# shepherdvovkes/sparse-matrix-multiplication-benchmark

Hardware: AMD Instinct MI355X
Metric: TCSC SpMM: effective G-add-ops/s + achieved HBM GB/s vs roofline, 1/2/4/8 GPU (higher is better)
Workload: dtype f32; 1 GPU; cfg4: M=4096 K=16384 N=16384, 98% ternary sparsity, fp32, tcsc_gemm_prelu; M=4096, K=16384, N=16384, variant=prelu_basic, columns_per_gpu=16384, nnz_per_gpu=5369271, parallelism=column-shard x1 (strong), no collective, rows_per_gpu=4096

## Files before the change

### include/tcsc_gpu.h

```cpp
#ifndef TCSC_AMD_TCSC_GPU_H
#define TCSC_AMD_TCSC_GPU_H

#include <stddef.h>
#include "sparse/tcsc.h"

#ifdef __cplusplus
extern "C" {
#endif

enum tcsc_variant {
    TCSC_VARIANT_BASIC = 0,
    TCSC_VARIANT_OPTIMIZED = 1,
    TCSC_VARIANT_PRELU_BASIC = 2,
    TCSC_VARIANT_PRELU_SEPARATE = 3,
    TCSC_VARIANT_PRELU_ONTHEGO = 4,
    TCSC_VARIANT_SPARSE_GEMM = 5
};

enum tcsc_status {
    TCSC_OK = 0,
    TCSC_E_ARG = 1,
    TCSC_E_HIP = 2,
    TCSC_E_NOMEM = 3,
    TCSC_E_NODEV = 4
// ... 39 lines not shown
int tcsc_gpu_plan_get_info(const tcsc_gpu_plan *plan, tcsc_gpu_plan_info *info);

enum tcsc_path {
    TCSC_PATH_GATHER = 0,
    TCSC_PATH_FUSED = 1,
    TCSC_PATH_MFMA = 2,
    TCSC_PATH_SMALL = 3,
    TCSC_PATH_DECODE = 4
};
int tcsc_gpu_launch_info(const tcsc_gpu_plan *plan, int M, int *path, int *slices);

int tcsc_gpu_launch_combine(const tcsc_gpu_plan *plan, int M, int *in_launch);

int tcsc_gpu_launch_geometry(const tcsc_gpu_plan *plan, int M, int *cols_per_wave);
int tcsc_gpu_wide_pays(int M, int ncols, int num_cus);

int tcsc_gpu_plan_reserve(tcsc_gpu_plan *plan, int max_M);
void tcsc_gpu_plan_destroy(tcsc_gpu_plan *plan);

#define TCSC_PATH_AUTO (-1)
int tcsc_gpu_plan_workspace(const tcsc_gpu_plan *plan, int M, int path, size_t *need, size_t *reserved);

int tcsc_gpu_sgemm(const tcsc_gpu_plan *plan, const float *dX, const float *dB,
                   float *dY, int M, int ldy, int variant, float a,
                   void *stream);

int tcsc_gpu_prepare_x(const tcsc_gpu_plan *plan, const float *dX, int M, void *stream);
int tcsc_gpu_sgemm_prepared(const tcsc_gpu_plan *plan, const float *dB, float *dY, int M, int ldy,
                            int variant, float a, void *stream);

// ... 98 lines not shown
```

### sparse-matrix-multiplication-benchmark_amd/csrc/tcsc_api.cpp

```cpp
#include <hip/hip_runtime.h>
#include <rocblas/rocblas.h>

#include <algorithm>
#include <cstdarg>
#include <cstdint>
#include <cstdio>
#include <cstdlib>
#include <cstring>
#include <memory>
#include <mutex>
#include <string>
#include <unordered_map>
#include <vector>

#include "../../include/sparse/tcsc.h"
#include "../../include/tcsc_gpu.h"
#include "tcsc_plan.h"

struct tcsc_gpu_plan {
    int device = 0;
    int rows = 0, cols = 0, col_begin = 0;
    long long n_pos = 0, n_neg = 0;
    int n_chunks = 0, n_groups = 0;
    long long n_entries = 0;
// ... 10 lines not shown
    size_t mfma_bytes = 0;
    int8_t* w8 = nullptr;
    size_t i8_bytes = 0;
    uint32_t* w2 = nullptr;
    size_t w2_bytes = 0;
    int *ccq = nullptr, *crq = nullptr;
    size_t csc_bytes = 0;
    int mfma_min_M = 0;
    unsigned* csync = nullptr;
    mutable bool csync_dirty = false;
    int num_cus = 0;
    int2* ent_w = nullptr;
    int* sptr_w = nullptr;
    long long n_entries_w = 0;
    int n_groups_w = 0;
    size_t wide_bytes = 0;
    float* tbias = nullptr;
    size_t tbias_bytes = 0;
    bool packed = false;
};

namespace {
thread_local std::string g_last_error;
}

namespace tcsc {

void set_error(const char* fmt, ...) {
    char buf[512];
    va_list ap;
// ... 560 lines not shown
    if (f == tcsc::kWideCW) return true;
    if (f == tcsc::kCW) return false;
    const int top = std::min(max_M, kMaxLaunchRows);
    for (long long M = tcsc::kTM; M < top + tcsc::kTM; M += tcsc::kTM)
        if (wide_pays((int)std::min<long long>(M, top), p->cols, p->num_cus)) return true;
    return false;
}

int build_wide(tcsc_gpu_plan* p) {
    if (p->ent_w) return TCSC_OK;
    DeviceGuard dg(p->device);
    hipStream_t st = nullptr;
    const int nch = p->n_chunks, G = p->n_groups, ncols = p->cols, Gw = tcsc::wide_groups_for(ncols);
    const long long nc = (long long)nch * ncols, ng = (long long)nch * Gw;
    if (nch <= 0 || ng + 1 > 0x7fffffffLL) return TCSC_OK;
    DevBuf cnt, cptr, gcnt, tmp;
    size_t tb1 = 0, tb2 = 0;
    HIP_TRY(tcsc::plan_scan_tmp_bytes(nc + 1, &tb1));
    HIP_TRY(tcsc::plan_scan_tmp_bytes(ng + 1, &tb2));
    const size_t tb = std::max(tb1, tb2);
    int* sptr_w = nullptr;
    if (cnt.alloc((size_t)(nc + 1) * sizeof(int)) != hipSuccess || cptr.alloc((size_t)(nc + 1) * sizeof(int)) != hipSuccess ||
        gcnt.alloc((size_t)(ng + 1) * sizeof(int)) != hipSuccess || tmp.alloc(tb) != hipSuccess ||
        hipMalloc(&sptr_w, (size_t)(ng + 1) * sizeof(int)) != hipSuccess) {
        (void)hipGetLastError();
        return TCSC_OK;
    }
    std::unique_ptr<int, void (*)(int*)> sptr_guard(sptr_w, [](int* q) { (void)hipFree(q); });
    HIP_TRY(hipDeviceSynchronize());
    HIP_TRY(tcsc::wide_counts(p->ent, p->sptr, G, nch, ncols, Gw, cnt.as<int>(), cptr.as<int>(), gcnt.as<int>(), sptr_w,
                              tmp.p, tb, st));
    int total = 0;
    HIP_TRY(hipMemcpyAsync(&total, sptr_w + ng, sizeof(int), hipMemcpyDeviceToHost, st));
    HIP_TRY(hipStreamSynchronize(st));
    int2* ent_w = nullptr;
    if (hipMalloc(&ent_w, (size_t)(total + tcsc::kEntGuard) * sizeof(int2)) != hipSuccess) {
        (void)hipGetLastError();
        return TCSC_OK;
    }
    hipError_t e = tcsc::wide_fill(p->ent, p->sptr, G, nch, ncols, Gw, cptr.as<int>(), sptr_w, ent_w, total, st);
    if (e == hipSuccess) e = hipStreamSynchronize(st);
    if (e != hipSuccess) {
        (void)hipFree(ent_w);
        return hip_fail(e, "build_wide");
    }
    p->ent_w = ent_w;
    p->sptr_w = sptr_guard.release();
    p->n_entries_w = total;
    p->n_groups_w = Gw;
    p->wide_bytes = (size_t)(ng + 1) * sizeof(int) + (size_t)(total + tcsc::kEntGuard) * sizeof(int2);
    return TCSC_OK;
}

int launch_geo(const tcsc_gpu_plan* p, int M, int slices, int forced_slices, const char* who) {
    const int f = geo_override();
    if (f == tcsc::kWideCW) {
        if (p->order != TCSC_ORDER_FAST || forced_slices > 1) {
            if (who)
                set_error("%s: TCSC_GEO=22 needs the fast order and an unsplit K (order %s, %d slices forced)", who,
                          p->order == TCSC_ORDER_FAST ? "fast" : "reference", forced_slices);
            return -1;
        }
        if (p->rows <= 0) return tcsc::kCW;
        if (!p->ent_w) {
            if (who)
// ... 214 lines not shown
        g.ent2 = p->chain_neg->ent;
        g.sptr2 = p->chain_neg->sptr;
        g.n_entries2 = p->chain_neg->n_entries;
    }
    g.n_groups = p->n_groups;
    g.a = a;
    g.slices = r.slices;
    g.combine = r.combine;
    g.stage = stage;
    if (stage != 1) {
        if (r.geo < 0) return TCSC_E_ARG;
        if (r.geo == tcsc::kWideCW) {
            g.geo = r.geo;
            g.ent = p->ent_w;
            g.sptr = p->sptr_w;
            g.n_entries = p->n_entries_w;
            g.n_groups = p->n_groups_w;
            g.slices = 1;
            g.combine = 0;
        }
    }
    if (pins.plan_ws && p->csync) {
        if (p->csync_dirty) {
            HIP_TRY(hipMemsetAsync(p->csync, 0, tcsc::kCombineBytes, static_cast<hipStream_t>(stream)));
            p->csync_dirty = false;
        }
        g.ccnt = p->csync;
        g.combine_giveup = combine_giveup_knob();
    }
    g.bias_first = (g.order == 1 && variant == TCSC_VARIANT_BASIC);
// ... 459 lines not shown
    g_order = order == TCSC_ORDER_REFERENCE ? TCSC_ORDER_REFERENCE : TCSC_ORDER_FAST;
}

int tcsc_gpu_get_order(void) { return current_order(); }

void tcsc_gpu_plan_destroy(tcsc_gpu_plan* p) {
    if (!p) return;
    DeviceGuard dg(p->device);
    if (p->ent) (void)hipFree(p->ent);
    if (p->sptr) (void)hipFree(p->sptr);
    if (p->ws) (void)hipFree(p->ws);
    if (p->csync) (void)hipFree(p->csync);
    if (p->tbias) (void)hipFree(p->tbias);
    if (p->ent_w) (void)hipFree(p->ent_w);
    if (p->sptr_w) (void)hipFree(p->sptr_w);
    free_mfma(p);
    free_csc(p);
    tcsc_gpu_plan_destroy(p->chain_pos);
    tcsc_gpu_plan_destroy(p->chain_neg);
    delete p;
}

int tcsc_gpu_plan_reserve(tcsc_gpu_plan* p, int max_M) {
    if (!p || max_M < 0) {
        set_error("tcsc_gpu_plan_reserve: bad arguments");
        return TCSC_E_ARG;
    }
    const size_t want = reserve_bytes(p, max_M);
    if (!p->csync && p->rows > 0 && p->order == TCSC_ORDER_FAST && !p->packed) {
        DeviceGuard dg(p->device);
// ... 48 lines not shown
}

int tcsc_gpu_launch_info(const tcsc_gpu_plan* p, int M, int* path, int* slices) {
    return launch_info_impl("tcsc_gpu_launch_info", p, M, path, slices, kF32);
}

int tcsc_gpu_launch_info_bf16(const tcsc_gpu_plan* p, int M, int* path, int* slices) {
    return launch_info_impl("tcsc_gpu_launch_info_bf16", p, M, path, slices, kBf16);
}

int tcsc_gpu_launch_info_i8(const tcsc_gpu_plan* p, int M, int* path, int* slices) {
    return launch_info_impl("tcsc_gpu_launch_info_i8", p, M, path, slices, kI8);
}

int tcsc_gpu_wide_pays(int M, int ncols, int num_cus) { return wide_pays(M, ncols, num_cus) ? 1 : 0; }

int tcsc_gpu_launch_geometry(const tcsc_gpu_plan* p, int M, int* cols_per_wave) {
    if (!p || M < 0 || !cols_per_wave) {
        set_error("tcsc_gpu_launch_geometry: bad arguments");
        return TCSC_E_ARG;
    }
    if (refuse_packed(p, "tcsc_gpu_launch_geometry")) return TCSC_E_ARG;
    *cols_per_wave = 0;
    const Route r = plan_route(p, M, kF32, "tcsc_gpu_launch_geometry");
    if (r.path != TCSC_PATH_GATHER) return TCSC_OK;
    if (r.geo < 0) return TCSC_E_ARG;
    *cols_per_wave = r.geo;
    return TCSC_OK;
}

// ... 601 lines not shown
```

### sparse-matrix-multiplication-benchmark_amd/csrc/tcsc_internal.h

```cpp
#pragma once
#include <hip/hip_runtime.h>
#include <stddef.h>
#include <stdint.h>

namespace tcsc {

constexpr int kTM = 256;
#ifndef TCSC_TK
#define TCSC_TK 48
#endif
#ifndef TCSC_NBUF
#define TCSC_NBUF 3
#endif
constexpr int kTK = TCSC_TK;
constexpr int kNBuf = TCSC_NBUF;
constexpr int kRowBytes = kTM * 4;
constexpr int kBufRows = kTK + 1;
#ifndef TCSC_WAVES
#define TCSC_WAVES 16
#endif
#ifndef TCSC_CW
#define TCSC_CW 16
#endif
#ifndef TCSC_BATCH
// ... 60 lines not shown
constexpr int kDmaPerWave = kTK / kDmaWaves;
static_assert(kDmaWaves <= kWaves && kTK % kDmaWaves == 0, "each DMA wave moves the same number of rows");
static_assert(kLdsBytes <= 160 * 1024, "LDS");
static_assert(kNBuf >= 2 && kNBuf <= 5, "ring of 2 (DMA(c+1) before gather(c)) or n >= 3 (DMA(c+n-1) after it)");

static_assert(4 * kCW <= 255, "slot index must fit the 8-bit gpr_idx field");
static_assert(64 * 16 <= 1024, "lane byte offset (16*lane) must fit the 10 low address bits");

constexpr int kWideCW = 22;
constexpr int kWideBatch = 3;
constexpr int kWideWgCols = kWaves * kWideCW;
__host__ __device__ constexpr int wide_group_col0(int g) { return (g / kWaves) * kWideWgCols + (g % kWaves) * kWideCW; }
__host__ __device__ constexpr int wide_groups_for(int ncols) {
    return (ncols / kWideWgCols) * kWaves + (ncols % kWideWgCols + kWideCW - 1) / kWideCW;
}

struct PlanDev {
    int rows = 0;
    int ncols = 0;
    int col_begin = 0;
    long long n_pos = 0, n_neg = 0;
    const int* csp = nullptr;
    const int* csn = nullptr;
    const int* rip = nullptr;
    const int* rin = nullptr;
};

struct PlanOut {
    int n_chunks = 0;
    int n_groups = 0;
// ... 18 lines not shown
struct GemmArgs {
    const void* X = nullptr;
    int xtype = kF32;
    const float* Xscale = nullptr;
    float* XT = nullptr;
    int M = 0, K = 0;
    const int2* ent = nullptr;
    const int* sptr = nullptr;
    long long n_entries = 0;
    int order = 0;
    const int2* ent2 = nullptr;
    const int* sptr2 = nullptr;
    long long n_entries2 = 0;
    int n_groups = 0;
    int geo = kCW;
    int ncols = 0;
    const float* B = nullptr;
    float* Y = nullptr;
    int ldy = 0;
    float a = 0.f;
    bool bias_first = false;
    bool prelu = false;
    float* ws = nullptr;
    size_t ws_bytes = 0;
    int slices = 1;
    int combine = 0;
    int stage = 0;
    unsigned* ccnt = nullptr;
    int combine_giveup = 0;
};
// ... 2 lines not shown
           ((reinterpret_cast<uintptr_t>(g.Y) | reinterpret_cast<uintptr_t>(g.ws) | reinterpret_cast<uintptr_t>(g.B)) & 15) == 0;
}
constexpr int kMaxLaunchRows = 1 << 22;

hipError_t plan_scan_tmp_bytes(long long n, size_t* bytes);
hipError_t plan_counts(const PlanDev& in, PlanOut& out, hipStream_t st);
hipError_t plan_fill(const PlanDev& in, PlanOut& out, hipStream_t st);
int choose_slices(int M, int ncols, int K, long long nnz, int n_groups, size_t ws_bytes, int force);
int combine_mode(int slices, long long wgs, long long tiles, long long slab_floats, int num_cus, bool have_words,
                 bool vec);
int normalized_slices(int K, int slices);
void pf_stream_params(long long n_entries, int n_groups, int n_chunks, int* dist, int* lines);
size_t workspace_bytes(int M, int ncols, int slices);
size_t xt_bytes(int M, int K);
hipError_t launch_gemm(const GemmArgs& g, hipStream_t st);
hipError_t wide_counts(const int2* ent, const int* sptr, int G, int nch, int ncols, int Gw, int* cnt, int* cptr,
                       int* gcnt, int* sptr_w, void* tmp, size_t tmp_bytes, hipStream_t st);
hipError_t wide_fill(const int2* ent, const int* sptr, int G, int nch, int ncols, int Gw, const int* cptr,
                     const int* sptr_w, int2* ent_w, long long n_entries, hipStream_t st);
hipError_t launch_stream_wide(const GemmArgs& g, hipStream_t st);
int dense_tile_rows(int rows);
hipError_t dense_to_tcsc_counts(const float* D, int rows, int cols, int* cp, int* cn, int* totp, int* totn,
                                hipStream_t st);
hipError_t dense_to_tcsc_fill(const float* D, int rows, int cols, const int* csp, const int* csn, const int* op,
                              const int* on, int* rip, int* rin, hipStream_t st);
hipError_t launch_bias_act(float* Y, int M, int N, int ldy, const float* B, bool prelu, float a, hipStream_t st);
hipError_t exclusive_scan_i32(const int* in, int* out, int n, void* tmp, size_t tmp_bytes, hipStream_t st);
hipError_t check_index_device(const int* cs, const int* ri, int col_begin, int ncols, int rows, int n_total,
                              int* d_flag, hipStream_t st);
hipError_t rebase_offsets(const int* cs, int col_begin, int ncols, int* out, hipStream_t st);
hipError_t sort_columns_tmp_bytes(int n, int ncols, size_t* bytes);
hipError_t sort_columns(const int* in, int* out, int n, int ncols, const int* off, void* tmp, size_t tmp_bytes,
                        hipStream_t st);
int ldxt_for(int M);
// ... 125 lines not shown
```

### sparse-matrix-multiplication-benchmark_amd/csrc/tcsc_wide.hip

```cpp
#include <hip/hip_runtime.h>
#include <hipcub/hipcub.hpp>
#include <stdint.h>

#include "tcsc_internal.h"

namespace tcsc {

#include "gather_asm_w22.inc"

static_assert(TCSCW_GEN_CW == kWideCW && TCSCW_GEN_BATCH == kWideBatch, "generated loop geometry");
static_assert(TCSCW_GEN_CAP + kHdr <= kEntGuard, "stream prefetch stays inside the entry guard");
static_assert(TCSCW_GEN_HDR == 2 * kHdr, "generated loop and plan agree on the chunk header");
static_assert(TCSCW_GEN_BUDGET == (512 / kWavesPerSimd) / 8 * 8, "generated loop VGPR budget");
static_assert(TCSCW_GEN_TAIL == 1, "the wide streams are unpadded");
static_assert(TCSCW_GEN_TOUCH == 0 && TCSCW_GEN_PF == 0, "no scalar-cache touches in the wide loop");
static_assert(4 * kWideCW <= 255, "slot index must fit the 8-bit gpr_idx field");
static_assert(kWaves == 16 && kTK % 16 == 0 && kNBuf >= 3, "the wide kernel's DMA split and ring");

namespace {

typedef float f32x32_t __attribute__((ext_vector_type(32)));
typedef float f32x16_t __attribute__((ext_vector_type(16)));
typedef float f32x8_t __attribute__((ext_vector_type(8)));
constexpr int kAccWidths[] = {TCSCW_ACC_WIDTHS};
// ... 81 lines not shown

__device__ __forceinline__ void xcd_tile_w(int bx, int by, int ncb, int nrt, int& cb, int& rt) {
    const int T = ncb * nrt;
    const int L = bx + ncb * by;
    const int q = T >> 3, r = T & 7, x = L & 7;
    const int Lg = (x < r ? x * (q + 1) : r * (q + 1) + (x - r) * q) + (L >> 3);
    cb = Lg % ncb;
    rt = Lg / ncb;
}

constexpr int kEpiRowsW = 64;
constexpr int kStrideW = kWideWgCols * 4 + 16;
constexpr int kLdsBytesW = kRingBytes + kPfScratch;
static_assert(kEpiRowsW * kStrideW <= kRingBytes, "the epilogue staging fits below the ring's end");
static_assert(kLdsBytesW <= 160 * 1024, "LDS");
static_assert((kWideCW * 4) % 8 == 0 && kWideCW % 2 == 0, "a wave's parked row piece is whole 8-byte pairs");
static_assert(kWideWgCols % 4 == 0 && kWideWgCols / 4 > 64 && kWideWgCols / 4 <= 128,
              "a tile row is 64 quads plus a second, partial set");

}

struct WideArgs {
    const float* XT;
    const int2* ent;
    const int* sptr;
    const float* Bias;
    float* Y;
    long long n_entries;
    int ldxt, M, G, ncols, nch, ldy;
    float a;
    int pf_dist, pf_lines;
};

template <bool BIAS_FIRST, bool PRELU>
__global__ void __launch_bounds__(kWaves * 64, kWavesPerSimd)
k_stream_w(const float* __restrict__ XT, const int2* __restrict__ ent, const int* __restrict__ sptr,
           const float* __restrict__ Bias0, float* __restrict__ Y0, long long n_entries, int ldxt, int M0, int G,
           int ncols0, int nch, int ldy0, float a0, int pf_dist, int pf_lines) {
    __shared__ __attribute__((aligned(16))) char lds[kLdsBytesW];
    const int lane = threadIdx.x & 63;
    const unsigned lane16 = 16u * lane;
    const int wave = __builtin_amdgcn_readfirstlane(threadIdx.x >> 6);
    int tcb, trt;
    xcd_tile_w(blockIdx.x, blockIdx.y, gridDim.x, gridDim.y, tcb, trt);
    const int g = tcb * kWaves + wave;
    const int m0 = trt * kTM;
    const bool active = g < G;

    AccW acc;
    acc_zero(acc);
    if (BIAS_FIRST && active) {
        const int cb = wide_group_col0(g) + lane;
        const float bv = (lane < kWideCW && cb < ncols0) ? Bias0[cb] : 0.f;
#pragma unroll
        for (int j = 0; j < kWideCW; ++j) {
            const float b = __shfl(bv, j);
#pragma unroll
            for (int r = 0; r < 4; ++r) acc_set(acc, 4 * j + r, b);
        }
    }

    if (threadIdx.x < 64 * kNBuf) {
        const int b = threadIdx.x >> 6;
        reinterpret_cast<float4*>(lds + (b * kBufRows + kTK) * kRowBytes)[lane] = make_float4(-0.f, -0.f, -0.f, -0.f);
    }

    if (nch > 0) {
        DmaW dma;
// ... 37 lines not shown
    __syncthreads();
    typedef __attribute__((address_space(4))) const WideArgs const_args;
    const_args* E = reinterpret_cast<const_args*>(reinterpret_cast<uintptr_t>(__builtin_amdgcn_kernarg_segment_ptr()));
    asm volatile("" : "+s"(E)::"memory");
    const float* __restrict__ Bias = E->Bias;
    float* __restrict__ Y = E->Y;
    const int M = E->M, ncols = E->ncols, ldy = E->ldy;
    const float a = E->a;
    int bx = blockIdx.x, by = blockIdx.y, gx = gridDim.x, gy = gridDim.y;
    asm volatile("" : "+s"(bx), "+s"(by), "+s"(gx), "+s"(gy));
    const int wave_e = __builtin_amdgcn_readfirstlane(threadIdx.x >> 6);
    int tcb_e, trt_e;
    xcd_tile_w(bx, by, gx, gy, tcb_e, trt_e);
    const bool active_e = tcb_e * kWaves + wave_e < E->G;
    const int m0_e = trt_e * kTM;
    constexpr int kLanesPerPass = kEpiRowsW / 4;
    constexpr int kQuads = kWideWgCols / 4;
    const int pcol = kWideCW * wave_e;
    const bool vec_ok = (ldy & 3) == 0 && ((reinterpret_cast<uintptr_t>(Y) & 15) == 0);
    float4 bq[2];
#pragma unroll
    for (int s = 0; s < 2; ++s) {
        const int col = tcb_e * kWideWgCols + 4 * (lane + 64 * s);
        const bool in = lane + 64 * s < kQuads;
        bq[s].x = (!BIAS_FIRST && in && col + 0 < ncols) ? Bias[col + 0] : 0.f;
        bq[s].y = (!BIAS_FIRST && in && col + 1 < ncols) ? Bias[col + 1] : 0.f;
        bq[s].z = (!BIAS_FIRST && in && col + 2 < ncols) ? Bias[col + 2] : 0.f;
        bq[s].w = (!BIAS_FIRST && in && col + 3 < ncols) ? Bias[col + 3] : 0.f;
    }
#pragma unroll
    for (int h = 0; h < kTM / kEpiRowsW; ++h) {
        if (active_e && lane / kLanesPerPass == h) {
            const int lh = lane % kLanesPerPass;
#pragma unroll
            for (int r = 0; r < 4; ++r) {
                const int R = 4 * lh + r;
#pragma unroll
                for (int j = 0; j < kWideCW; j += 2)
                    *reinterpret_cast<float2*>(lds + R * kStrideW + (pcol + j) * 4) =
                        make_float2(acc_get(acc, 4 * j + r), acc_get(acc, 4 * (j + 1) + r));
            }
        }
        __syncthreads();
#pragma unroll
        for (int i = 0; i < kEpiRowsW / kWaves; ++i) {
            const int R = wave_e + kWaves * i;
            const int row = m0_e + kEpiRowsW * h + R;
#pragma unroll
            for (int s = 0; s < 2; ++s) {
                const int q = lane + 64 * s;
                const int col = tcb_e * kWideWgCols + 4 * q;
                if (q < kQuads && row < M && col < ncols) {
                    float4 v = *reinterpret_cast<const float4*>(lds + R * kStrideW + q * 16);
                    if (!BIAS_FIRST) {
                        v.x += bq[s].x;
                        v.y += bq[s].y;
                        v.z += bq[s].z;
                        v.w += bq[s].w;
                    }
                    if (PRELU) {
                        v.x = (v.x < 0.0f) ? a * v.x : v.x;
                        v.y = (v.y < 0.0f) ? a * v.y : v.y;
// ... 41 lines not shown
        for (int e = 0; e < n; ++e) {
            const int w = ent[first + e].y;
            if (is_pad(w)) continue;
            const int s = (w & 0x3ff) >> 2;
            if (s != slot) {
                if (run) cnt[(long long)c * ncols + n0 + slot] = run;
                slot = s;
                run = 0;
            }
            ++run;
        }
        if (run) cnt[(long long)c * ncols + n0 + slot] = run;
    }
}

__global__ void k_wide_group_counts(const int* __restrict__ cptr, int ncols, int nch, int Gw, int* __restrict__ gcnt) {
    const long long total = (long long)nch * Gw;
    for (long long i = blockIdx.x * (long long)blockDim.x + threadIdx.x; i < total;
         i += (long long)gridDim.x * blockDim.x) {
        const int g = (int)(i / nch), c = (int)(i % nch);
        const int n0 = wide_group_col0(g), n1 = min(n0 + kWideCW, ncols);
        gcnt[i] = kHdr + cptr[(long long)c * ncols + n1] - cptr[(long long)c * ncols + n0];
    }
}

__global__ void k_wide_scatter(const int2* __restrict__ ent, const int* __restrict__ sptr, int G, int nch, int ncols,
                               const int* __restrict__ cptr, const int* __restrict__ sptr_w, int2* __restrict__ ent_w) {
    const long long total = (long long)G * nch;
    for (long long i = blockIdx.x * (long long)blockDim.x + threadIdx.x; i < total;
         i += (long long)gridDim.x * blockDim.x) {
        const int g = (int)(i / nch), c = (int)(i % nch);
        int first;
        const int n = stream_range(sptr, i, &first);
        const int n0 = group_col0(g);
        int rank = 0, slot = -1, base = 0, jw = 0;
        for (int e = 0; e < n; ++e) {
            const int2 v = ent[first + e];
            if (is_pad(v.y)) continue;
            const int s = (v.y & 0x3ff) >> 2;
            if (s != slot) {
                slot = s;
                rank = 0;
                const int col = n0 + s;
                const int gw = (col / kWideWgCols) * kWaves + (col % kWideWgCols) / kWideCW;
                jw = col - wide_group_col0(gw);
                base = sptr_w[(long long)gw * nch + c] + kHdr +
                       (cptr[(long long)c * ncols + col] - cptr[(long long)c * ncols + wide_group_col0(gw)]);
            }
            ent_w[base + rank++] = make_int2(v.x, (v.y & ~0x3ff) | (4 * jw));
        }
    }
}

__global__ void k_wide_headers(const int* __restrict__ sptr_w, int nch, int Gw, int2* __restrict__ ent_w,
                               long long n_entries) {
    const long long total = (long long)nch * Gw;
    for (long long i = blockIdx.x * (long long)blockDim.x + threadIdx.x; i < total;
         i += (long long)gridDim.x * blockDim.x) {
        const int s0 = sptr_w[i], s1 = sptr_w[i + 1];
        const int n = s1 - s0 - kHdr;
        ent_w[s0] = make_int2(n / kWideBatch, n % kWideBatch);
        ent_w[s0 + 1] = make_int2((s1 - s0) * (int)sizeof(int2), 0);
    }
    if (blockIdx.x == 0)
        for (int i = threadIdx.x; i < kEntGuard; i += blockDim.x)
            ent_w[n_entries + i] = i < kHdr ? make_int2(0, 0) : make_int2(0x3f800000, kTK << 10);
}

inline int grid_for(long long n, int block) {
    long long g = (n + block - 1) / block;
    if (g < 1) g = 1;
    if (g > 65535LL * 16) g = 65535LL * 16;
    return (int)g;
}

}

hipError_t wide_counts(const int2* ent, const int* sptr, int G, int nch, int ncols, int Gw, int* cnt, int* cptr,
                       int* gcnt, int* sptr_w, void* tmp, size_t tmp_bytes, hipStream_t st) {
    hipError_t e;
    const long long nc = (long long)nch * ncols, ng = (long long)nch * Gw;
    if ((e = hipMemsetAsync(cnt, 0, (size_t)(nc + 1) * sizeof(int), st)) != hipSuccess) return e;
    if ((e = hipMemsetAsync(gcnt + ng, 0, sizeof(int), st)) != hipSuccess) return e;
    hipLaunchKernelGGL(k_wide_col_counts, dim3(grid_for((long long)G * nch, 128)), dim3(128), 0, st, ent, sptr, G, nch,
                       ncols, cnt);
    if ((e = hipGetLastError()) != hipSuccess) return e;
    size_t tb = tmp_bytes;
    if ((e = hipcub::DeviceScan::ExclusiveSum(tmp, tb, cnt, cptr, (int)(nc + 1), st)) != hipSuccess) return e;
    hipLaunchKernelGGL(k_wide_group_counts, dim3(grid_for(ng, 256)), dim3(256), 0, st, cptr, ncols, nch, Gw, gcnt);
    if ((e = hipGetLastError()) != hipSuccess) return e;
    tb = tmp_bytes;
    return hipcub::DeviceScan::ExclusiveSum(tmp, tb, gcnt, sptr_w, (int)(ng + 1), st);
}

hipError_t wide_fill(const int2* ent, const int* sptr, int G, int nch, int ncols, int Gw, const int* cptr,
                     const int* sptr_w, int2* ent_w, long long n_entries, hipStream_t st) {
    hipLaunchKernelGGL(k_wide_scatter, dim3(grid_for((long long)G * nch, 128)), dim3(128), 0, st, ent, sptr, G, nch,
                       ncols, cptr, sptr_w, ent_w);
    hipError_t e = hipGetLastError();
    if (e != hipSuccess) return e;
    hipLaunchKernelGGL(k_wide_headers, dim3(grid_for((long long)nch * Gw, 256)), dim3(256), 0, st, sptr_w, nch, Gw,
                       ent_w, n_entries);
    return hipGetLastError();
}

hipError_t launch_stream_wide(const GemmArgs& g, hipStream_t st) {
    if (g.order != 0 || g.ent == nullptr) return hipErrorInvalidValue;
    const int nch = (g.K + kTK - 1) / kTK;
    const int ldxt = ldxt_for(g.M);
    dim3 grid((g.n_groups + kWaves - 1) / kWaves, (g.M + kTM - 1) / kTM, 1);
    dim3 block(kWaves * 64);
    int pfd = 0, pfl = 1;
    pf_stream_params(g.n_entries, g.n_groups, nch, &pfd, &pfl);
#define TCSC_LAUNCH_W(BF, PR)                                                                                         \
    hipLaunchKernelGGL((k_stream_w<BF, PR>), grid, block, 0, st, g.XT, g.ent, g.sptr, g.B, g.Y, g.n_entries, ldxt, g.M, \
                       g.n_groups, g.ncols, nch, g.ldy, g.a, pfd, pfl)
    if (g.bias_first) {
        if (g.prelu) TCSC_LAUNCH_W(true, true);
        else TCSC_LAUNCH_W(true, false);
    } else {
        if (g.prelu) TCSC_LAUNCH_W(false, true);
        else TCSC_LAUNCH_W(false, false);
    }
#undef TCSC_LAUNCH_W
    return hipGetLastError();
}

}
```

### sparse-matrix-multiplication-benchmark_amd/tcsc_amd/__init__.py

```python
from __future__ import annotations

import ctypes as C
import os
import subprocess

import numpy as np

PKG_DIR = os.path.dirname(os.path.dirname(os.path.abspath(__file__)))
LIB_PATH = os.environ.get("TCSC_AMD_LIB") or os.path.join(PKG_DIR, "lib", "libtcsc_amd.so")

VARIANTS = ("basic", "optimized", "prelu_basic", "prelu_separate", "prelu_onthego")
VARIANT_ID = {v: i for i, v in enumerate(VARIANTS)}
VARIANT_ID["sparse_gemm"] = 5
PRELU_VARIANTS = frozenset(VARIANTS[2:])

EXPORTED_SYMBOLS = (
    "tcsc_from_dense", "tcsc_sgemm_basic", "tcsc_sgemm_optimized", "tcsc_sgemm_prelu_basic",
    "tcsc_sgemm_prelu_optimized_separate", "tcsc_sgemm_prelu_optimized_onthego", "tcsc_free",
    "dense_random", "init_rand_dense", "init_rand_sparse", "compare", "gemm_basic", "gemm_prelu_basic",
    "tcsc_set_seed",
    "tcsc_gpu_device_count", "tcsc_gpu_plan_create", "tcsc_gpu_plan_create_device", "tcsc_gpu_plan_get_info",
    "tcsc_gpu_plan_reserve", "tcsc_gpu_plan_destroy", "tcsc_gpu_sgemm", "tcsc_gpu_prepare_x",
    "tcsc_gpu_sgemm_prepared", "tcsc_gpu_from_dense", "tcsc_gpu_dense_sgemm", "tcsc_gpu_last_error",
    "tcsc_gpu_cache_clear", "tcsc_gpu_num_shards", "tcsc_gpu_set_num_shards", "tcsc_gpu_set_order",
    "tcsc_gpu_get_order", "tcsc_gpu_launch_info", "tcsc_gpu_launch_combine", "tcsc_gpu_build_flags",
    "tcsc_gpu_plan_workspace", "tcsc_gpu_transpose_index", "tcsc_gpu_plan_create_transposed",
    "tcsc_gpu_plan_create_transposed_device", "tcsc_gpu_sgemm_t", "tcsc_gpu_prelu_backward",
    "tcsc_gpu_sgemm_bf16", "tcsc_gpu_launch_info_bf16",
    "tcsc_gpu_plan_enable_i8", "tcsc_gpu_plan_has_i8", "tcsc_gpu_sgemm_i8", "tcsc_gpu_launch_info_i8",
    "tcsc_gpu_quantize_rows_i8", "tcsc_gpu_workspace_bound_i8",
    "tcsc_gpu_plan_enable_w2", "tcsc_gpu_plan_has_w2", "tcsc_gpu_w2_image_bytes", "tcsc_gpu_decode_pays",
    "tcsc_gpu_launch_geometry", "tcsc_gpu_wide_pays",
    "tcsc_gpu_plan_create_packed", "tcsc_gpu_plan_create_packed_device", "tcsc_gpu_plan_is_packed",
    "tcsc_gpu_plan_copy_w2",
    "tcsc_gpu_plan_create_packed_image", "tcsc_gpu_plan_create_packed_image_device", "tcsc_gpu_w2_to_tcsc",
    "tcsc_gpu_w2_from_tcsc_host", "tcsc_gpu_w2_to_tcsc_host",
    "tcsc_gpu_quantize_rows_i8_bf16", "tcsc_gpu_sgemm_q8", "tcsc_gpu_launch_info_q8", "tcsc_gpu_quant_fuse_pays",
    "bcsr_from_dense", "bcsr_sgemm_basic", "bcsr_sgemm_prelu_basic", "bcsr_sgemm_avx", "bcsr_sgemm_prelu_avx",
    "bcsr_sgemm_avx2", "bcsr_free",
    "bcsr_gpu_plan_create", "bcsr_gpu_plan_stats", "bcsr_gpu_plan_reserve", "bcsr_gpu_plan_destroy",
    "bcsr_gpu_sgemm", "bcsr_gpu_prepare_x", "bcsr_gpu_sgemm_prepared",
    "tcsc_sparse_format", "tcsc_sparse_gemm", "tcsc_sparse_gemm_prelu", "tcsc_dense_gemm", "tcsc_dense_gemm_prelu",
)


class TcscError(RuntimeError):
    pass
# ... 55 lines not shown
              "tcsc_sgemm_prelu_optimized_onthego"):
        getattr(L, n).argtypes = [_f32p, P, _f32p, f, _f32p, i, i, i]
        getattr(L, n).restype = None
    L.tcsc_free.argtypes = [P]
    L.tcsc_free.restype = None
    L.tcsc_set_seed.argtypes = [C.c_ulonglong]
    L.tcsc_gpu_device_count.restype = i
    L.tcsc_gpu_last_error.restype = C.c_char_p
    L.tcsc_gpu_plan_create.argtypes = [P, i, i, i, vp, C.POINTER(vp)]
    L.tcsc_gpu_plan_create_device.argtypes = [i, i, vp, vp, vp, vp, i, i, i, vp, C.POINTER(vp)]
    L.tcsc_gpu_plan_get_info.argtypes = [vp, C.POINTER(plan_info_t)]
    L.tcsc_gpu_launch_info.argtypes = [vp, i, C.POINTER(i), C.POINTER(i)]
    L.tcsc_gpu_launch_combine.argtypes = [vp, i, C.POINTER(i)]
    L.tcsc_gpu_launch_geometry.argtypes = [vp, i, C.POINTER(i)]
    L.tcsc_gpu_wide_pays.argtypes = [i, i, i]
    L.tcsc_gpu_plan_reserve.argtypes = [vp, i]
    L.tcsc_gpu_plan_workspace.argtypes = [vp, i, i, C.POINTER(C.c_size_t), C.POINTER(C.c_size_t)]
    L.tcsc_gpu_plan_destroy.argtypes = [vp]
    L.tcsc_gpu_plan_destroy.restype = None
    L.tcsc_gpu_sgemm.argtypes = [vp, vp, vp, vp, i, i, i, f, vp]
    L.tcsc_gpu_sgemm_bf16.argtypes = [vp, vp, vp, vp, i, i, i, f, vp]
    L.tcsc_gpu_launch_info_bf16.argtypes = [vp, i, C.POINTER(i), C.POINTER(i)]
    L.tcsc_gpu_plan_enable_i8.argtypes = [vp, vp]
    L.tcsc_gpu_plan_has_i8.argtypes = [vp]
    L.tcsc_gpu_sgemm_i8.argtypes = [vp, vp, vp, vp, vp, i, i, i, f, vp]
    L.tcsc_gpu_launch_info_i8.argtypes = [vp, i, C.POINTER(i), C.POINTER(i)]
    L.tcsc_gpu_quantize_rows_i8.argtypes = [vp, i, i, vp, vp, vp]
    L.tcsc_gpu_workspace_bound_i8.argtypes = [i, i, i, C.POINTER(C.c_size_t), C.POINTER(C.c_size_t)]
    L.tcsc_gpu_plan_enable_w2.argtypes = [vp, vp]
    L.tcsc_gpu_plan_has_w2.argtypes = [vp]
# ... 407 lines not shown
        return self._launch_info("tcsc_gpu_launch_info_bf16", M)

    def launch_combine(self, M: int) -> bool:
        return self.combine_mode(M) is not None

    def combine_mode(self, M: int):
        v = C.c_int()
        _check(lib().tcsc_gpu_launch_combine(self.handle, int(M), C.byref(v)), "tcsc_gpu_launch_combine")
        return {2: "bands", 3: "pairwise", 4: "pairwise-split"}.get(v.value)

    def launch_geometry(self, M: int) -> int:
        v = C.c_int()
        _check(lib().tcsc_gpu_launch_geometry(self.handle, int(M), C.byref(v)), "tcsc_gpu_launch_geometry")
        return v.value

    def reserve(self, max_M: int) -> None:
        _check(lib().tcsc_gpu_plan_reserve(self.handle, int(max_M)), "tcsc_gpu_plan_reserve")

    PATH_ID = {None: -1, "gather": 0, "mfma": 2, "small": 3, "decode": 4}

    def workspace(self, M: int, path: str | None = None) -> tuple[int, int]:
        need, reserved = C.c_size_t(), C.c_size_t()
        _check(lib().tcsc_gpu_plan_workspace(self.handle, int(M), self.PATH_ID[path], C.byref(need),
                                             C.byref(reserved)), "tcsc_gpu_plan_workspace")
        return need.value, reserved.value

    def sgemm(self, X, B, Y, M: int, ldy: int, variant: str = "prelu_basic", a: float = 0.2,
              stream: int = 0) -> None:
        _check(lib().tcsc_gpu_sgemm(self.handle, C.c_void_p(_ptr(X)), C.c_void_p(_ptr(B)), C.c_void_p(_ptr(Y)),
                                    int(M), int(ldy), VARIANT_ID[variant], float(a), C.c_void_p(stream)),
# ... 229 lines not shown
```

Baseline: 19080 G-add-ops/s.

## Balance per-wave nonzero load in wide kernel by permuting columns within workgroups

Adds a plan-time greedy pass that reassigns columns among the waves of each wide workgroup so the per-chunk nonzero counts are more even. The permutation is kept only when it lowers the summed per-chunk maximum. The entry streams are rebuilt in the permuted order, and the epilogue uses the map to write results back to the original columns. The aim is to cut wave imbalance inside a workgroup, at the cost of scattered single-float LDS writes in the epilogue and an extra table lookup.

```diff
diff --git a/include/tcsc_gpu.h b/include/tcsc_gpu.h
--- a/include/tcsc_gpu.h
+++ b/include/tcsc_gpu.h
@@ -77,6 +77,8 @@
 
 int tcsc_gpu_launch_geometry(const tcsc_gpu_plan *plan, int M, int *cols_per_wave);
 int tcsc_gpu_wide_pays(int M, int ncols, int num_cus);
+int tcsc_gpu_plan_wide_stats(const tcsc_gpu_plan *plan, long long stats[4], unsigned short *map,
+                             size_t map_entries);
 
 int tcsc_gpu_plan_reserve(tcsc_gpu_plan *plan, int max_M);
 void tcsc_gpu_plan_destroy(tcsc_gpu_plan *plan);
diff --git a/sparse-matrix-multiplication-benchmark_amd/csrc/tcsc_api.cpp b/sparse-matrix-multiplication-benchmark_amd/csrc/tcsc_api.cpp
--- a/sparse-matrix-multiplication-benchmark_amd/csrc/tcsc_api.cpp
+++ b/sparse-matrix-multiplication-benchmark_amd/csrc/tcsc_api.cpp
@@ -48,6 +48,8 @@
     int* sptr_w = nullptr;
     long long n_entries_w = 0;
     int n_groups_w = 0;
+    unsigned short* wperm = nullptr;
+    long long wide_stats[4] = {0, 0, 0, 0};
     size_t wide_bytes = 0;
     float* tbias = nullptr;
     size_t tbias_bytes = 0;
@@ -638,31 +640,47 @@
     const int nch = p->n_chunks, G = p->n_groups, ncols = p->cols, Gw = tcsc::wide_groups_for(ncols);
     const long long nc = (long long)nch * ncols, ng = (long long)nch * Gw;
     if (nch <= 0 || ng + 1 > 0x7fffffffLL) return TCSC_OK;
-    DevBuf cnt, cptr, gcnt, tmp;
+    const char* bal_s = std::getenv("TCSC_WIDE_BALANCE");
+    const int balance = bal_s && std::atoi(bal_s) == 0 ? 0 : 1;
+    const size_t nmap = (size_t)tcsc::wide_blocks_for(ncols) * tcsc::kWideWgCols;
+    DevBuf cnt, cptr, gcnt, tmp, loads, winv, wstats;
     size_t tb1 = 0, tb2 = 0;
     HIP_TRY(tcsc::plan_scan_tmp_bytes(nc + 1, &tb1));
     HIP_TRY(tcsc::plan_scan_tmp_bytes(ng + 1, &tb2));
     const size_t tb = std::max(tb1, tb2);
     int* sptr_w = nullptr;
+    unsigned short* wperm = nullptr;
     if (cnt.alloc((size_t)(nc + 1) * sizeof(int)) != hipSuccess || cptr.alloc((size_t)(nc + 1) * sizeof(int)) != hipSuccess ||
         gcnt.alloc((size_t)(ng + 1) * sizeof(int)) != hipSuccess || tmp.alloc(tb) != hipSuccess ||
+        loads.alloc(nmap / tcsc::kWideCW * nch * sizeof(int)) != hipSuccess ||
+        winv.alloc((size_t)ncols * sizeof(unsigned short)) != hipSuccess ||
+        wstats.alloc(4 * sizeof(unsigned long long)) != hipSuccess ||
         hipMalloc(&sptr_w, (size_t)(ng + 1) * sizeof(int)) != hipSuccess) {
         (void)hipGetLastError();
         return TCSC_OK;
     }
     std::unique_ptr<int, void (*)(int*)> sptr_guard(sptr_w, [](int* q) { (void)hipFree(q); });
+    if (hipMalloc(&wperm, nmap * sizeof(unsigned short)) != hipSuccess) {
+        (void)hipGetLastError();
+        return TCSC_OK;
+    }
+    std::unique_ptr<unsigned short, void (*)(unsigned short*)> wperm_guard(wperm, [](unsigned short* q) { (void)hipFree(q); });
     HIP_TRY(hipDeviceSynchronize());
-    HIP_TRY(tcsc::wide_counts(p->ent, p->sptr, G, nch, ncols, Gw, cnt.as<int>(), cptr.as<int>(), gcnt.as<int>(), sptr_w,
+    HIP_TRY(tcsc::wide_counts(p->ent, p->sptr, G, nch, ncols, Gw, balance, cnt.as<int>(), cptr.as<int>(), gcnt.as<int>(),
+                              sptr_w, loads.as<int>(), wperm, winv.as<unsigned short>(), wstats.as<unsigned long long>(),
                               tmp.p, tb, st));
     int total = 0;
+    unsigned long long stats[4] = {0, 0, 0, 0};
     HIP_TRY(hipMemcpyAsync(&total, sptr_w + ng, sizeof(int), hipMemcpyDeviceToHost, st));
+    HIP_TRY(hipMemcpyAsync(stats, wstats.p, sizeof stats, hipMemcpyDeviceToHost, st));
     HIP_TRY(hipStreamSynchronize(st));
     int2* ent_w = nullptr;
     if (hipMalloc(&ent_w, (size_t)(total + tcsc::kEntGuard) * sizeof(int2)) != hipSuccess) {
         (void)hipGetLastError();
         return TCSC_OK;
     }
-    hipError_t e = tcsc::wide_fill(p->ent, p->sptr, G, nch, ncols, Gw, cptr.as<int>(), sptr_w, ent_w, total, st);
+    hipError_t e = tcsc::wide_fill(p->ent, p->sptr, G, nch, ncols, Gw, cptr.as<int>(), winv.as<unsigned short>(), sptr_w,
+                                   ent_w, total, st);
     if (e == hipSuccess) e = hipStreamSynchronize(st);
     if (e != hipSuccess) {
         (void)hipFree(ent_w);
@@ -670,9 +688,12 @@
     }
     p->ent_w = ent_w;
     p->sptr_w = sptr_guard.release();
+    p->wperm = wperm_guard.release();
+    for (int i = 0; i < 4; ++i) p->wide_stats[i] = (long long)stats[i];
     p->n_entries_w = total;
     p->n_groups_w = Gw;
-    p->wide_bytes = (size_t)(ng + 1) * sizeof(int) + (size_t)(total + tcsc::kEntGuard) * sizeof(int2);
+    p->wide_bytes = (size_t)(ng + 1) * sizeof(int) + (size_t)(total + tcsc::kEntGuard) * sizeof(int2) +
+                    nmap * sizeof(unsigned short);
     return TCSC_OK;
 }
 
@@ -917,6 +938,7 @@
             g.geo = r.geo;
             g.ent = p->ent_w;
             g.sptr = p->sptr_w;
+            g.wperm = p->wperm;
             g.n_entries = p->n_entries_w;
             g.n_groups = p->n_groups_w;
             g.slices = 1;
@@ -1406,6 +1428,7 @@
     if (p->tbias) (void)hipFree(p->tbias);
     if (p->ent_w) (void)hipFree(p->ent_w);
     if (p->sptr_w) (void)hipFree(p->sptr_w);
+    if (p->wperm) (void)hipFree(p->wperm);
     free_mfma(p);
     free_csc(p);
     tcsc_gpu_plan_destroy(p->chain_pos);
@@ -1484,6 +1507,29 @@
 }
 
 int tcsc_gpu_wide_pays(int M, int ncols, int num_cus) { return wide_pays(M, ncols, num_cus) ? 1 : 0; }
+
+int tcsc_gpu_plan_wide_stats(const tcsc_gpu_plan* p, long long stats[4], unsigned short* map, size_t map_entries) {
+    if (!p || (!stats && !map)) {
+        set_error("tcsc_gpu_plan_wide_stats: bad arguments");
+        return TCSC_E_ARG;
+    }
+    if (!p->ent_w || !p->wperm) {
+        set_error("tcsc_gpu_plan_wide_stats: the plan has no wide streams (tcsc_gpu_plan_reserve builds them)");
+        return TCSC_E_ARG;
+    }
+    if (stats)
+        for (int i = 0; i < 4; ++i) stats[i] = p->wide_stats[i];
+    if (map) {
+        const size_t nmap = (size_t)tcsc::wide_blocks_for(p->cols) * tcsc::kWideWgCols;
+        if (map_entries != nmap) {
+            set_error("tcsc_gpu_plan_wide_stats: the map has %zu entries, not %zu", nmap, map_entries);
+            return TCSC_E_ARG;
+        }
+        DeviceGuard dg(p->device);
+        HIP_TRY(hipMemcpy(map, p->wperm, nmap * sizeof(unsigned short), hipMemcpyDeviceToHost));
+    }
+    return TCSC_OK;
+}
 
 int tcsc_gpu_launch_geometry(const tcsc_gpu_plan* p, int M, int* cols_per_wave) {
     if (!p || M < 0 || !cols_per_wave) {
diff --git a/sparse-matrix-multiplication-benchmark_amd/csrc/tcsc_internal.h b/sparse-matrix-multiplication-benchmark_amd/csrc/tcsc_internal.h
--- a/sparse-matrix-multiplication-benchmark_amd/csrc/tcsc_internal.h
+++ b/sparse-matrix-multiplication-benchmark_amd/csrc/tcsc_internal.h
@@ -98,6 +98,7 @@
 __host__ __device__ constexpr int wide_groups_for(int ncols) {
     return (ncols / kWideWgCols) * kWaves + (ncols % kWideWgCols + kWideCW - 1) / kWideCW;
 }
+__host__ __device__ constexpr int wide_blocks_for(int ncols) { return (ncols + kWideWgCols - 1) / kWideWgCols; }
 
 struct PlanDev {
     int rows = 0;
@@ -146,6 +147,7 @@
     long long n_entries2 = 0;
     int n_groups = 0;
     int geo = kCW;
+    const unsigned short* wperm = nullptr;
     int ncols = 0;
     const float* B = nullptr;
     float* Y = nullptr;
@@ -178,10 +180,11 @@
 size_t workspace_bytes(int M, int ncols, int slices);
 size_t xt_bytes(int M, int K);
 hipError_t launch_gemm(const GemmArgs& g, hipStream_t st);
-hipError_t wide_counts(const int2* ent, const int* sptr, int G, int nch, int ncols, int Gw, int* cnt, int* cptr,
-                       int* gcnt, int* sptr_w, void* tmp, size_t tmp_bytes, hipStream_t st);
+hipError_t wide_counts(const int2* ent, const int* sptr, int G, int nch, int ncols, int Gw, int balance, int* cnt,
+                       int* cptr, int* gcnt, int* sptr_w, int* loads, unsigned short* wperm, unsigned short* winv,
+                       unsigned long long* wstats, void* tmp, size_t tmp_bytes, hipStream_t st);
 hipError_t wide_fill(const int2* ent, const int* sptr, int G, int nch, int ncols, int Gw, const int* cptr,
-                     const int* sptr_w, int2* ent_w, long long n_entries, hipStream_t st);
+                     const unsigned short* winv, const int* sptr_w, int2* ent_w, long long n_entries, hipStream_t st);
 hipError_t launch_stream_wide(const GemmArgs& g, hipStream_t st);
 int dense_tile_rows(int rows);
 hipError_t dense_to_tcsc_counts(const float* D, int rows, int cols, int* cp, int* cn, int* totp, int* totn,
diff --git a/sparse-matrix-multiplication-benchmark_amd/csrc/tcsc_wide.hip b/sparse-matrix-multiplication-benchmark_amd/csrc/tcsc_wide.hip
--- a/sparse-matrix-multiplication-benchmark_amd/csrc/tcsc_wide.hip
+++ b/sparse-matrix-multiplication-benchmark_amd/csrc/tcsc_wide.hip
@@ -119,7 +119,7 @@
 constexpr int kLdsBytesW = kRingBytes + kPfScratch;
 static_assert(kEpiRowsW * kStrideW <= kRingBytes, "the epilogue staging fits below the ring's end");
 static_assert(kLdsBytesW <= 160 * 1024, "LDS");
-static_assert((kWideCW * 4) % 8 == 0 && kWideCW % 2 == 0, "a wave's parked row piece is whole 8-byte pairs");
+static_assert(kWideCW <= 64 && kWideWgCols <= 65535, "one lane per slot reads its 16-bit column position");
 static_assert(kWideWgCols % 4 == 0 && kWideWgCols / 4 > 64 && kWideWgCols / 4 <= 128,
               "a tile row is 64 quads plus a second, partial set");
 
@@ -131,6 +131,7 @@
     const int* sptr;
     const float* Bias;
     float* Y;
+    const unsigned short* wperm;
     long long n_entries;
     int ldxt, M, G, ncols, nch, ldy;
     float a;
@@ -140,8 +141,9 @@
 template <bool BIAS_FIRST, bool PRELU>
 __global__ void __launch_bounds__(kWaves * 64, kWavesPerSimd)
 k_stream_w(const float* __restrict__ XT, const int2* __restrict__ ent, const int* __restrict__ sptr,
-           const float* __restrict__ Bias0, float* __restrict__ Y0, long long n_entries, int ldxt, int M0, int G,
-           int ncols0, int nch, int ldy0, float a0, int pf_dist, int pf_lines) {
+           const float* __restrict__ Bias0, float* __restrict__ Y0, const unsigned short* __restrict__ wperm0,
+           long long n_entries, int ldxt, int M0, int G, int ncols0, int nch, int ldy0, float a0, int pf_dist,
+           int pf_lines) {
     __shared__ __attribute__((aligned(16))) char lds[kLdsBytesW];
     const int lane = threadIdx.x & 63;
     const unsigned lane16 = 16u * lane;
@@ -155,8 +157,8 @@
     AccW acc;
     acc_zero(acc);
     if (BIAS_FIRST && active) {
-        const int cb = wide_group_col0(g) + lane;
-        const float bv = (lane < kWideCW && cb < ncols0) ? Bias0[cb] : 0.f;
+        const int cb = lane < kWideCW ? tcb * kWideWgCols + wperm0[tcb * kWideWgCols + wave * kWideCW + lane] : ncols0;
+        const float bv = cb < ncols0 ? Bias0[cb] : 0.f;
 #pragma unroll
         for (int j = 0; j < kWideCW; ++j) {
             const float b = __shfl(bv, j);
@@ -224,9 +226,13 @@
     xcd_tile_w(bx, by, gx, gy, tcb_e, trt_e);
     const bool active_e = tcb_e * kWaves + wave_e < E->G;
     const int m0_e = trt_e * kTM;
-    constexpr int kLanesPerPass = kEpiRowsW / 4;
+    static_assert(kEpiRowsW == 64 && kTM == 4 * kEpiRowsW, "a pass parks one of each lane's four rows");
     constexpr int kQuads = kWideWgCols / 4;
-    const int pcol = kWideCW * wave_e;
+    const unsigned short* __restrict__ wperm = E->wperm;
+    const int posv = lane < kWideCW ? wperm[tcb_e * kWideWgCols + wave_e * kWideCW + lane] : 0;
+    int pos[kWideCW];
+#pragma unroll
+    for (int j = 0; j < kWideCW; ++j) pos[j] = __builtin_amdgcn_readlane(posv, j);
     const bool vec_ok = (ldy & 3) == 0 && ((reinterpret_cast<uintptr_t>(Y) & 15) == 0);
     float4 bq[2];
 #pragma unroll
@@ -240,22 +246,16 @@
     }
 #pragma unroll
     for (int h = 0; h < kTM / kEpiRowsW; ++h) {
-        if (active_e && lane / kLanesPerPass == h) {
-            const int lh = lane % kLanesPerPass;
-#pragma unroll
-            for (int r = 0; r < 4; ++r) {
-                const int R = 4 * lh + r;
-#pragma unroll
-                for (int j = 0; j < kWideCW; j += 2)
-                    *reinterpret_cast<float2*>(lds + R * kStrideW + (pcol + j) * 4) =
-                        make_float2(acc_get(acc, 4 * j + r), acc_get(acc, 4 * (j + 1) + r));
-            }
+        if (active_e) {
+#pragma unroll
+            for (int j = 0; j < kWideCW; ++j)
+                *reinterpret_cast<float*>(lds + lane * kStrideW + pos[j] * 4) = acc_get(acc, 4 * j + h);
         }
         __syncthreads();
 #pragma unroll
         for (int i = 0; i < kEpiRowsW / kWaves; ++i) {
             const int R = wave_e + kWaves * i;
-            const int row = m0_e + kEpiRowsW * h + R;
+            const int row = m0_e + 4 * R + h;
 #pragma unroll
             for (int s = 0; s < 2; ++s) {
                 const int q = lane + 64 * s;
@@ -327,6 +327,149 @@
     }
 }
 
+template <typename T>
+__device__ __forceinline__ T wave_sum(T v) {
+#pragma unroll
+    for (int o = 32; o > 0; o >>= 1) v += __shfl_xor(v, o);
+    return v;
+}
+
+__global__ void __launch_bounds__(kWaves * 64)
+k_wide_balance(const int* __restrict__ cnt, int ncols, int nch, int balance, int* L0, unsigned short* __restrict__ wperm,
+               unsigned short* __restrict__ winv) {
+    __shared__ int tot[kWideWgCols];
+    __shared__ unsigned short order[kWideWgCols], cand[kWideWgCols];
+    __shared__ int nslot[kWaves];
+    __shared__ unsigned long long score[kWaves], red[2][kWaves];
+    __shared__ int best_s, keep_s;
+    const int tid = threadIdx.x, nt = blockDim.x, lane = tid & 63, wave = tid >> 6;
+    const int c0 = blockIdx.x * kWideWgCols;
+    unsigned short* perm = wperm + (size_t)blockIdx.x * kWideWgCols;
+    if (!balance || c0 + kWideWgCols > ncols) {
+        for (int i = tid; i < kWideWgCols; i += nt) {
+            perm[i] = (unsigned short)i;
+            if (c0 + i < ncols) winv[c0 + i] = (unsigned short)i;
+        }
+        return;
+    }
+    const int* blk = cnt + c0;
+    int* L = L0 + (size_t)blockIdx.x * kWaves * nch;
+    for (int col = tid; col < kWideWgCols; col += nt) {
+        int s = 0;
+        for (int c = 0; c < nch; ++c) s += blk[(size_t)c * ncols + col];
+        tot[col] = s;
+    }
+    for (int i = tid; i < kWaves * nch; i += nt) L[i] = 0;
+    if (tid < kWaves) nslot[tid] = 0;
+    __syncthreads();
+    for (int i = tid; i < kWideWgCols; i += nt) {
+        int r = 0;
+        for (int j = 0; j < kWideWgCols; ++j) r += (tot[j] > tot[i] || (tot[j] == tot[i] && j < i)) ? 1 : 0;
+        order[r] = (unsigned short)i;
+    }
+    __syncthreads();
+    for (int step = 0; step < kWideWgCols; ++step) {
+        const int col = order[step];
+        const int* cc = blk + col;
+        unsigned long long s = 0;
+        if (nslot[wave] < kWideCW)
+            for (int c = lane; c < nch; c += 64)
+                s += (unsigned long long)L[(size_t)wave * nch + c] * (unsigned long long)cc[(size_t)c * ncols];
+        s = wave_sum(s);
+        if (lane == 0) score[wave] = s;
+        __syncthreads();
+        if (tid == 0) {
+            int best = -1;
+            for (int w = 0; w < kWaves; ++w)
+                if (nslot[w] < kWideCW && (best < 0 || score[w] < score[best])) best = w;
+            cand[best * kWideCW + nslot[best]++] = (unsigned short)col;
+            best_s = best;
+        }
+        __syncthreads();
+        const int bw = best_s;
+        for (int c = tid; c < nch; c += nt) L[(size_t)bw * nch + c] += cc[(size_t)c * ncols];
+        __syncthreads();
+    }
+    unsigned long long sg = 0, si = 0;
+    for (int c = tid; c < nch; c += nt) {
+        int mg = 0, mi = 0;
+        for (int w = 0; w < kWaves; ++w) {
+            mg = max(mg, L[(size_t)w * nch + c]);
+            int s = 0;
+            for (int j = 0; j < kWideCW; ++j) s += blk[(size_t)c * ncols + w * kWideCW + j];
+            mi = max(mi, s);
+        }
+        sg += (unsigned long long)mg;
+        si += (unsigned long long)mi;
+    }
+    sg = wave_sum(sg);
+    si = wave_sum(si);
+    if (lane == 0) {
+        red[0][wave] = sg;
+        red[1][wave] = si;
+    }
+    __syncthreads();
+    if (tid == 0) {
+        unsigned long long g = 0, i = 0;
+        for (int w = 0; w < kWaves; ++w) {
+            g += red[0][w];
+            i += red[1][w];
+        }
+        keep_s = g < i ? 1 : 0;
+    }
+    __syncthreads();
+    const bool keep = keep_s != 0;
+    for (int i = tid; i < kWideWgCols; i += nt) {
+        const int v = keep ? cand[i] : i;
+        perm[i] = (unsigned short)v;
+        winv[c0 + v] = (unsigned short)i;
+    }
+}
+
+__global__ void k_wide_permute_counts(const int* __restrict__ cnt, const unsigned short* __restrict__ wperm, int ncols,
+                                      int nch, int* __restrict__ cntp) {
+    const long long total = (long long)nch * ncols;
+    for (long long i = blockIdx.x * (long long)blockDim.x + threadIdx.x; i <= total;
+         i += (long long)gridDim.x * blockDim.x) {
+        if (i == total) {
+            cntp[i] = 0;
+            continue;
+        }
+        const int q = (int)(i % ncols), b0 = q / kWideWgCols * kWideWgCols;
+        cntp[i] = cnt[i - q + b0 + wperm[q]];
+    }
+}
+
+__global__ void k_wide_stats(const int* __restrict__ cnt, const unsigned short* __restrict__ wperm, int ncols, int nch,
+                             unsigned long long* __restrict__ st) {
+    const int c0 = blockIdx.x * kWideWgCols;
+    const unsigned short* perm = wperm + (size_t)blockIdx.x * kWideWgCols;
+    unsigned long long v[4] = {0, 0, 0, 0};
+    for (int c = threadIdx.x; c < nch; c += blockDim.x) {
+        const int* row = cnt + (size_t)c * ncols + c0;
+        int mi = 0, mp = 0;
+        for (int w = 0; w < kWaves; ++w) {
+            int si = 0, sp = 0;
+            for (int j = 0; j < kWideCW; ++j) {
+                const int ci = w * kWideCW + j, cp = perm[ci];
+                si += c0 + ci < ncols ? row[ci] : 0;
+                sp += c0 + cp < ncols ? row[cp] : 0;
+            }
+            mi = max(mi, si);
+            mp = max(mp, sp);
+            v[2] += si > TCSCW_GEN_CAP ? 1 : 0;
+            v[3] += sp > TCSCW_GEN_CAP ? 1 : 0;
+        }
+        v[0] += (unsigned long long)mi;
+        v[1] += (unsigned long long)mp;
+    }
+#pragma unroll
+    for (int k = 0; k < 4; ++k) {
+        const unsigned long long s = wave_sum(v[k]);
+        if ((threadIdx.x & 63) == 0 && s) atomicAdd(st + k, s);
+    }
+}
+
 __global__ void k_wide_group_counts(const int* __restrict__ cptr, int ncols, int nch, int Gw, int* __restrict__ gcnt) {
     const long long total = (long long)nch * Gw;
     for (long long i = blockIdx.x * (long long)blockDim.x + threadIdx.x; i < total;
@@ -338,7 +481,8 @@
 }
 
 __global__ void k_wide_scatter(const int2* __restrict__ ent, const int* __restrict__ sptr, int G, int nch, int ncols,
-                               const int* __restrict__ cptr, const int* __restrict__ sptr_w, int2* __restrict__ ent_w) {
+                               const int* __restrict__ cptr, const unsigned short* __restrict__ winv,
+                               const int* __restrict__ sptr_w, int2* __restrict__ ent_w) {
     const long long total = (long long)G * nch;
     for (long long i = blockIdx.x * (long long)blockDim.x + threadIdx.x; i < total;
          i += (long long)gridDim.x * blockDim.x) {
@@ -355,10 +499,11 @@
                 slot = s;
                 rank = 0;
                 const int col = n0 + s;
-                const int gw = (col / kWideWgCols) * kWaves + (col % kWideWgCols) / kWideCW;
-                jw = col - wide_group_col0(gw);
+                const int p = col / kWideWgCols * kWideWgCols + winv[col];
+                const int gw = (p / kWideWgCols) * kWaves + (p % kWideWgCols) / kWideCW;
+                jw = p - wide_group_col0(gw);
                 base = sptr_w[(long long)gw * nch + c] + kHdr +
-                       (cptr[(long long)c * ncols + col] - cptr[(long long)c * ncols + wide_group_col0(gw)]);
+                       (cptr[(long long)c * ncols + p] - cptr[(long long)c * ncols + wide_group_col0(gw)]);
             }
             ent_w[base + rank++] = make_int2(v.x, (v.y & ~0x3ff) | (4 * jw));
         }
@@ -389,17 +534,28 @@
 
 }
 
-hipError_t wide_counts(const int2* ent, const int* sptr, int G, int nch, int ncols, int Gw, int* cnt, int* cptr,
-                       int* gcnt, int* sptr_w, void* tmp, size_t tmp_bytes, hipStream_t st) {
+hipError_t wide_counts(const int2* ent, const int* sptr, int G, int nch, int ncols, int Gw, int balance, int* cnt,
+                       int* cptr, int* gcnt, int* sptr_w, int* loads, unsigned short* wperm, unsigned short* winv,
+                       unsigned long long* wstats, void* tmp, size_t tmp_bytes, hipStream_t st) {
     hipError_t e;
     const long long nc = (long long)nch * ncols, ng = (long long)nch * Gw;
+    const int nblk = wide_blocks_for(ncols);
     if ((e = hipMemsetAsync(cnt, 0, (size_t)(nc + 1) * sizeof(int), st)) != hipSuccess) return e;
     if ((e = hipMemsetAsync(gcnt + ng, 0, sizeof(int), st)) != hipSuccess) return e;
+    if ((e = hipMemsetAsync(wstats, 0, 4 * sizeof(unsigned long long), st)) != hipSuccess) return e;
     hipLaunchKernelGGL(k_wide_col_counts, dim3(grid_for((long long)G * nch, 128)), dim3(128), 0, st, ent, sptr, G, nch,
                        ncols, cnt);
     if ((e = hipGetLastError()) != hipSuccess) return e;
+    hipLaunchKernelGGL(k_wide_balance, dim3(nblk), dim3(kWaves * 64), 0, st, cnt, ncols, nch, balance, loads, wperm,
+                       winv);
+    if ((e = hipGetLastError()) != hipSuccess) return e;
+    hipLaunchKernelGGL(k_wide_stats, dim3(nblk), dim3(256), 0, st, cnt, wperm, ncols, nch, wstats);
+    if ((e = hipGetLastError()) != hipSuccess) return e;
+    hipLaunchKernelGGL(k_wide_permute_counts, dim3(grid_for(nc + 1, 256)), dim3(256), 0, st, cnt, wperm, ncols, nch,
+                       cptr);
+    if ((e = hipGetLastError()) != hipSuccess) return e;
     size_t tb = tmp_bytes;
-    if ((e = hipcub::DeviceScan::ExclusiveSum(tmp, tb, cnt, cptr, (int)(nc + 1), st)) != hipSuccess) return e;
+    if ((e = hipcub::DeviceScan::ExclusiveSum(tmp, tb, cptr, cptr, (int)(nc + 1), st)) != hipSuccess) return e;
     hipLaunchKernelGGL(k_wide_group_counts, dim3(grid_for(ng, 256)), dim3(256), 0, st, cptr, ncols, nch, Gw, gcnt);
     if ((e = hipGetLastError()) != hipSuccess) return e;
     tb = tmp_bytes;
@@ -407,9 +563,9 @@
 }
 
 hipError_t wide_fill(const int2* ent, const int* sptr, int G, int nch, int ncols, int Gw, const int* cptr,
-                     const int* sptr_w, int2* ent_w, long long n_entries, hipStream_t st) {
+                     const unsigned short* winv, const int* sptr_w, int2* ent_w, long long n_entries, hipStream_t st) {
     hipLaunchKernelGGL(k_wide_scatter, dim3(grid_for((long long)G * nch, 128)), dim3(128), 0, st, ent, sptr, G, nch,
-                       ncols, cptr, sptr_w, ent_w);
+                       ncols, cptr, winv, sptr_w, ent_w);
     hipError_t e = hipGetLastError();
     if (e != hipSuccess) return e;
     hipLaunchKernelGGL(k_wide_headers, dim3(grid_for((long long)nch * Gw, 256)), dim3(256), 0, st, sptr_w, nch, Gw,
@@ -418,16 +574,16 @@
 }
 
 hipError_t launch_stream_wide(const GemmArgs& g, hipStream_t st) {
-    if (g.order != 0 || g.ent == nullptr) return hipErrorInvalidValue;
+    if (g.order != 0 || g.ent == nullptr || g.wperm == nullptr) return hipErrorInvalidValue;
     const int nch = (g.K + kTK - 1) / kTK;
     const int ldxt = ldxt_for(g.M);
     dim3 grid((g.n_groups + kWaves - 1) / kWaves, (g.M + kTM - 1) / kTM, 1);
     dim3 block(kWaves * 64);
     int pfd = 0, pfl = 1;
     pf_stream_params(g.n_entries, g.n_groups, nch, &pfd, &pfl);
-#define TCSC_LAUNCH_W(BF, PR)                                                                                         \
-    hipLaunchKernelGGL((k_stream_w<BF, PR>), grid, block, 0, st, g.XT, g.ent, g.sptr, g.B, g.Y, g.n_entries, ldxt, g.M, \
-                       g.n_groups, g.ncols, nch, g.ldy, g.a, pfd, pfl)
+#define TCSC_LAUNCH_W(BF, PR)                                                                                \
+    hipLaunchKernelGGL((k_stream_w<BF, PR>), grid, block, 0, st, g.XT, g.ent, g.sptr, g.B, g.Y, g.wperm, g.n_entries, \
+                       ldxt, g.M, g.n_groups, g.ncols, nch, g.ldy, g.a, pfd, pfl)
     if (g.bias_first) {
         if (g.prelu) TCSC_LAUNCH_W(true, true);
         else TCSC_LAUNCH_W(true, false);
diff --git a/sparse-matrix-multiplication-benchmark_amd/tcsc_amd/__init__.py b/sparse-matrix-multiplication-benchmark_amd/tcsc_amd/__init__.py
--- a/sparse-matrix-multiplication-benchmark_amd/tcsc_amd/__init__.py
+++ b/sparse-matrix-multiplication-benchmark_amd/tcsc_amd/__init__.py
@@ -30,7 +30,7 @@
     "tcsc_gpu_plan_enable_i8", "tcsc_gpu_plan_has_i8", "tcsc_gpu_sgemm_i8", "tcsc_gpu_launch_info_i8",
     "tcsc_gpu_quantize_rows_i8", "tcsc_gpu_workspace_bound_i8",
     "tcsc_gpu_plan_enable_w2", "tcsc_gpu_plan_has_w2", "tcsc_gpu_w2_image_bytes", "tcsc_gpu_decode_pays",
-    "tcsc_gpu_launch_geometry", "tcsc_gpu_wide_pays",
+    "tcsc_gpu_launch_geometry", "tcsc_gpu_wide_pays", "tcsc_gpu_plan_wide_stats",
     "tcsc_gpu_plan_create_packed", "tcsc_gpu_plan_create_packed_device", "tcsc_gpu_plan_is_packed",
     "tcsc_gpu_plan_copy_w2",
     "tcsc_gpu_plan_create_packed_image", "tcsc_gpu_plan_create_packed_image_device", "tcsc_gpu_w2_to_tcsc",
@@ -116,6 +116,7 @@
     L.tcsc_gpu_launch_combine.argtypes = [vp, i, C.POINTER(i)]
     L.tcsc_gpu_launch_geometry.argtypes = [vp, i, C.POINTER(i)]
     L.tcsc_gpu_wide_pays.argtypes = [i, i, i]
+    L.tcsc_gpu_plan_wide_stats.argtypes = [vp, C.POINTER(C.c_longlong), vp, C.c_size_t]
     L.tcsc_gpu_plan_reserve.argtypes = [vp, i]
     L.tcsc_gpu_plan_workspace.argtypes = [vp, i, i, C.POINTER(C.c_size_t), C.POINTER(C.c_size_t)]
     L.tcsc_gpu_plan_destroy.argtypes = [vp]
@@ -553,6 +554,14 @@
         _check(lib().tcsc_gpu_launch_geometry(self.handle, int(M), C.byref(v)), "tcsc_gpu_launch_geometry")
         return v.value
 
+    def wide_stats(self) -> dict:
+        st = (C.c_longlong * 4)()
+        nblk = (self.info()["cols"] + 351) // 352
+        m = np.empty((nblk, 16, 22), np.uint16)
+        _check(lib().tcsc_gpu_plan_wide_stats(self.handle, st, C.c_void_p(m.ctypes.data), m.size),
+               "tcsc_gpu_plan_wide_stats")
+        return dict(max_identity=st[0], max_balanced=st[1], long_identity=st[2], long_balanced=st[3], map=m)
+
     def reserve(self, max_M: int) -> None:
         _check(lib().tcsc_gpu_plan_reserve(self.handle, int(max_M)), "tcsc_gpu_plan_reserve")
 
```

New measurement: 19500 G-add-ops/s, median of 6. 2.2% higher.
